# kepengxu/PGTFormer

Hardware: NVIDIA H100
Metric: clips_per_s (higher is better)
Workload: dtype bf16

## Files before the change

### pgtformer_b200/csrc/gemm_tc.cu

```cuda
#include <cudaTypedefs.h>
#include <cstdio>
#include <cstdlib>

#include "common.cuh"
#include "tmap.cuh"
#include "ptx.cuh"
#include "epi_common.cuh"

namespace pgt {

constexpr int BM = 128;
constexpr int BK = 64;
constexpr int EPI_WARPS = 8;
constexpr int GEMM_THREADS = EPI_WARPS * 32 + 128;
constexpr int PRODUCER_WARP = EPI_WARPS;
constexpr int DMA_WARP = EPI_WARPS + 1;
constexpr int CONSUMER_REGS = 232;
constexpr int PRODUCER_REGS = 40;
static_assert(2 * 128 * CONSUMER_REGS + 128 * PRODUCER_REGS <= 65536, "register file");
constexpr int XCH_LD = 68;
constexpr int XCH_BYTES = BM * XCH_LD * 4;
constexpr int XCH_WG_LD = 36;
constexpr int XCH_WG_BYTES = BM * XCH_WG_LD * 4;
constexpr int EPI_BAR = 1;
constexpr int PP_XCH_BAR = 2;
constexpr int PP_MMA_BAR = 4;
constexpr int PP_EPI_BAR = 6;
constexpr int A_STAGE_BYTES = BM * BK * 2;
constexpr int PANEL_BYTES = BM * 128;
template <int BN>
constexpr int staging_slots() { return BN == 256 ? 2 : 4; }
constexpr int PREFETCH_TILES = 2;

enum { MODE_LINEAR = 0, MODE_CONV_S1 = 1, MODE_CONV_S2 = 2 };

struct GemmParams {
  int mode;
  int M, N, K;
  int num_kb, m_tiles, n_tiles;
  int F, H, W;
  int tw, th, tn, tiles_x, tiles_y;
  int cin_blocks, ksize, pad_lo, cin_ld;
  int pad_x, pad_y;
  long long o_sx, o_sy, o_sf;
  int b_resident;
  int fast_epi;
  int has_res_map;
  const float* bias;
  int act, epi_mode;
  float* gn_stats;
  int gn_cpg;
  int ntaps, tap_kw, tap_oy, tap_ox;
  int gn_tpf;
  int gn_fstride;
  int relu_after_res;
  const void* residual;
  int ldr, res_dtype;
  const void* aux;
  int ldaux;
  float sft_w;
  void* out;
  int ldo, out_dtype, out_layout;
  double flops;
};

template <int BN>
struct GemmCfg {
  static constexpr int B_STAGE_BYTES = BN * BK * 2;
  static constexpr int STAGE_BYTES = A_STAGE_BYTES + B_STAGE_BYTES;
  static constexpr int SLOTS = staging_slots<BN>();
  static constexpr int STAGING_BYTES = SLOTS * PANEL_BYTES;
  static constexpr int BUDGET = 232448 - 1024  - STAGING_BYTES - XCH_BYTES - 256 ;
  static constexpr int STAGES = (BUDGET / STAGE_BYTES) > 6 ? 6 : (BUDGET / STAGE_BYTES);
  static constexpr int SMEM_BYTES = STAGES * STAGE_BYTES + STAGING_BYTES + XCH_BYTES + 256 + 1024;
  static_assert(SMEM_BYTES <= 232448, "gemm smem budget");
};

__device__ __forceinline__ void tile_mn(const GemmParams& p, int tile, int& m_blk, int& n_blk) {
  n_blk = tile % p.n_tiles;
  m_blk = tile / p.n_tiles;
}


__device__ __forceinline__ void decode_conv_tile(const GemmParams& p, int m_blk, int& n0, int& y0, int& x0) {
  const int tx = m_blk % p.tiles_x;
  const int t2 = m_blk / p.tiles_x;
  const int ty = t2 % p.tiles_y;
  const int tf = t2 / p.tiles_y;
  x0 = tx * p.tw;
  y0 = ty * p.th;
  n0 = tf * p.tn;
}

template <int N>
__device__ __forceinline__ void act_chunk(float (&f)[N], int act) {
  switch (act) {
    case PGT_ACT_GELU:
#pragma unroll
// ... 363 lines not shown
          mbar_wait_spin(&ctx.res_bar[pos], (k >> 1) & 1);
          const int col0 = col_base + pnl * PW + half * 32;
          uint32_t v[32];
          smem_row_32(xrow + half * 32, v);
          float4 nb[8];
          epi_finish<true>(p, v, bias_vec ? p.bias + col0 : nullptr, stg + pos * 2 * PANEL_BYTES, r, half, esize, true,
                           gn_ptr(col0), col0, nb, false);
          fence_proxy_async();
          mbar_arrive(&ctx.slot_ready[pos]);
          ++k;
        }
      } else {
        for (int pp = 0; pp < 64 / PW; ++pp) {
          const int pnl = g * (64 / PW) + pp;
          if (pnl >= npan) break;
          const int pos = k & (SLOTS - 1);
          const bool mine = (nsub == 2) || ((pnl & 1) == half);
          const int sb = (nsub == 2) ? half : 0;
          const int col0 = col_base + pnl * PW + sb * 32;
          float4 b[8];
          const bool pre = BN < 256 && bias_vec;
          if (mine && pre) {
            const float4* gb = reinterpret_cast<const float4*>(p.bias + col0);
#pragma unroll
            for (int q = 0; q < 8; ++q) b[q] = __ldg(gb + q);
          }
          mbar_wait_spin(&ctx.res_bar[pos], (k >> SLOT_SHIFT) & 1);
          if (mine) {
            uint32_t v[32];
            smem_row_32(xrow + pnl * PW + sb * 32 - g * 64, v);
            epi_finish<false>(p, v, bias_vec && !pre ? p.bias + col0 : nullptr, stg + pos * PANEL_BYTES, r, sb, esize,
                              p.has_res_map != 0, gn_ptr(col0), col0, b, pre);
          }
          fence_proxy_async();
          mbar_arrive(&ctx.slot_ready[pos]);
          ++k;
        }
      }
    } else {
      const int c0 = g * 64 + half * 32;
      if (drow.valid) {
#pragma unroll 1
        for (int sc16 = 0; sc16 < 32; sc16 += 16) {
          const int col0 = col_base + c0 + sc16;
          if (col0 >= p.N) break;
          epi_direct16(p, drow, xrow + half * 32 + sc16, col0);
        }
      }
      __syncwarp();
    }
  });
}

template <int BN>
__device__ __forceinline__ void epilogue_tile_wg(const GemmParams& p, const EpiCtx& ctx, int wq, int bar, int tile, int k,
                                                 const float (&acc)[2][BN / 2]) {
  const int lane = lane_id();
  const int r = wq * 32 + lane;
  const int esize = (p.out_dtype == PGT_BF16) ? 2 : 4;
  const ItemStream<BN> is(p, 0);
  const int nsub = is.PW / 32;
  constexpr int SLOTS = staging_slots<BN>();
  constexpr int SLOT_SHIFT = SLOTS == 4 ? 2 : 1;
  const bool sft = SLOTS == 4 && p.epi_mode == PGT_EPI_SFT;
  const bool bias_vec = p.bias != nullptr && (p.N % 32) == 0;
  const float* xrow = ctx.xch + r * XCH_WG_LD;

  int n_blk, m_blk;
  tile_mn(p, tile, m_blk, n_blk);
  const int col_base = n_blk * BN;
  const int npan = p.fast_epi ? is.panels_in_tile(tile) : 0;
  const uint32_t stg = smem_u32(ctx.staging) + r * 128;
  const DirectRow drow = p.fast_epi ? DirectRow{false, 0, 0, 0, 0} : direct_row(p, m_blk, r);

  static_for<0, BN / 32>([&](auto cc) {
    constexpr int c = decltype(cc)::value;
    const int pnl = c / nsub, sub = c - pnl * nsub;
    if (p.fast_epi && pnl >= npan) return;
    const int col0 = col_base + c * 32;
    if (col0 < p.N) {
      named_bar_sync(bar, 128);
      acc_to_smem<c * 32, 32>(acc[0], ctx.xch, XCH_WG_LD, wq, lane);
      acc_to_smem<c * 32, 32>(acc[1], ctx.xch + 64 * XCH_WG_LD, XCH_WG_LD, wq, lane);
      named_bar_sync(bar, 128);
    }
    if (p.fast_epi) {
      const int item = k + pnl;
      const int pos = sft ? (item & 1) : (item & (SLOTS - 1));
      if (sub == 0) mbar_wait_spin(&ctx.res_bar[pos], sft ? ((item >> 1) & 1) : ((item >> SLOT_SHIFT) & 1));
      if (col0 < p.N) {
        uint32_t v[32];
        smem_row_32(xrow, v);
        float4 nb[8];
        if (sft)
          epi_finish<true>(p, v, bias_vec ? p.bias + col0 : nullptr, stg + pos * 2 * PANEL_BYTES, r, sub, esize, true,
                           gn_stats_ptr(p, m_blk, wq, col0), col0, nb, false);
        else
          epi_finish<false>(p, v, bias_vec ? p.bias + col0 : nullptr, stg + pos * PANEL_BYTES, r, sub, esize,
                            p.has_res_map != 0, gn_stats_ptr(p, m_blk, wq, col0), col0, nb, false);
      }
      if (sub == nsub - 1) {
        fence_proxy_async();
        mbar_arrive(&ctx.slot_ready[pos]);
      }
    } else if (col0 < p.N) {
      if (drow.valid) {
#pragma unroll 1
        for (int sc16 = 0; sc16 < 32; sc16 += 16) {
          if (col0 + sc16 >= p.N) break;
          epi_direct16(p, drow, xrow + sc16, col0 + sc16);
        }
      }
      __syncwarp();
    }
  });
}

__device__ __forceinline__ void release_stage(uint64_t* bar, int lane) {
  __syncwarp();
  if (lane == 0) mbar_arrive(bar);
}

template <int BN>
__global__ void __launch_bounds__(GEMM_THREADS, 1)
gemm_tc_kernel(const __grid_constant__ CUtensorMap tmA, const __grid_constant__ CUtensorMap tmB,
               const __grid_constant__ CUtensorMap tmO, const __grid_constant__ CUtensorMap tmR,
               const __grid_constant__ CUtensorMap tmX, const GemmParams p) {
  using Cfg = GemmCfg<BN>;
  constexpr int STAGES = Cfg::STAGES;
  extern __shared__ uint8_t smem_raw[];
  uint8_t* smem = reinterpret_cast<uint8_t*>((reinterpret_cast<uintptr_t>(smem_raw) + 1023) & ~uintptr_t(1023));
  uint8_t* smem_a = smem;
  uint8_t* smem_b = smem + STAGES * A_STAGE_BYTES;
  uint8_t* staging = smem + STAGES * Cfg::STAGE_BYTES;
  float* xch = reinterpret_cast<float*>(staging + Cfg::STAGING_BYTES);
  uint64_t* bars = reinterpret_cast<uint64_t*>(staging + Cfg::STAGING_BYTES + XCH_BYTES);
  uint64_t* full_bar = bars;
  uint64_t* empty_bar = bars + STAGES;
  uint64_t* res_bar = bars + 2 * STAGES;
  uint64_t* slot_ready = res_bar + Cfg::SLOTS;

  const int warp = threadIdx.x >> 5;
  const int lane = threadIdx.x & 31;
  const int num_tiles = p.m_tiles * p.n_tiles;

  if (warp == PRODUCER_WARP && lane == 0) {
    tma_prefetch_desc(&tmA);
    tma_prefetch_desc(&tmB);
    if (p.fast_epi) tma_prefetch_desc(&tmO);
    if (p.has_res_map) tma_prefetch_desc(&tmR);
    if (p.fast_epi && p.epi_mode == PGT_EPI_SFT) tma_prefetch_desc(&tmX);
    for (int i = 0; i < STAGES; ++i) {
      mbar_init(&full_bar[i], 1);
      mbar_init(&empty_bar[i], EPI_WARPS);
    }
    for (int i = 0; i < Cfg::SLOTS; ++i) {
      mbar_init(&res_bar[i], 1);
      mbar_init(&slot_ready[i], EPI_WARPS * 32);
    }
    fence_barrier_init();
  }
  __syncthreads();

// ... 36 lines not shown
            tma_load_2d(dst_b, &tmB, &full_bar[stage], kb * BK, n_blk * BN);
          }
          __syncwarp();
          if (++stage == STAGES) { stage = 0; phase ^= 1; }
        }
      }
      for (int i = 0; i < STAGES; ++i) {
        mbar_wait(&empty_bar[stage], phase ^ 1);
        if (++stage == STAGES) { stage = 0; phase ^= 1; }
      }
    } else if (warp == DMA_WARP) {
      const EpiCtx ctx{staging, xch, res_bar, slot_ready};
      epilogue_dma_loop<BN>(p, ctx, tmO, tmR, tmX, lane, num_tiles);
    }
  } else {
    setmaxnreg_inc<CONSUMER_REGS>();
    const EpiCtx ctx{staging, xch, res_bar, slot_ready};
    const int wg = warp >> 2;
    const uint32_t a_rows = smem_u32(smem_a) + wg * 64 * 128;
    const uint32_t b_base = smem_u32(smem_b);
    int stage = 0;
    uint32_t phase = 0;
    int k = 0;
    for (int tile = blockIdx.x; tile < num_tiles; tile += gridDim.x) {
      float acc[BN / 2];
      int prev = -1;
      for (int kb = 0; kb < p.num_kb; ++kb) {
        mbar_wait_spin(&full_bar[stage], phase);
        const uint64_t da = wgmma_desc_k_sw128(a_rows + stage * A_STAGE_BYTES);
        const uint64_t db = wgmma_desc_k_sw128(b_base + stage * Cfg::B_STAGE_BYTES);
        wgmma_fence();
#pragma unroll
        for (int kk = 0; kk < BK / 16; ++kk)
          wgmma_bf16<BN>(acc, da + 2 * kk, db + 2 * kk, (kb | kk) != 0 ? 1u : 0u);
        wgmma_commit();
        wgmma_wait<1>();
        if (prev >= 0) release_stage(&empty_bar[prev], lane);
        prev = stage;
        if (++stage == STAGES) { stage = 0; phase ^= 1; }
      }
      wgmma_wait<0>();
      release_stage(&empty_bar[prev], lane);
      epilogue_tile<BN>(p, ctx, warp, lane, tile, k, acc);
    }
  }
}


constexpr int HALO_TW = 8, HALO_TH = 16;
constexpr int HALO_PITCH = (HALO_TW + 2) * 128;
constexpr int HALO_A_BYTES = (HALO_TH + 2) * HALO_PITCH;
constexpr int HALO_A_STRIDE = ((HALO_A_BYTES + 1023) / 1024) * 1024;

template <int BN>
struct HaloCfg {
  static constexpr int B_BYTES = BN * 128;
  static constexpr int A_STAGES = 2;
  static constexpr int B_STAGES = (BN == 64) ? 9 : 4;
  static constexpr int SLOTS = staging_slots<BN>();
  static constexpr int STAGING_BYTES = SLOTS * PANEL_BYTES;
  static constexpr int XCH = 2 * XCH_WG_BYTES;
  static constexpr int SMEM_BYTES = A_STAGES * HALO_A_STRIDE + B_STAGES * B_BYTES + STAGING_BYTES + XCH + 512 + 1024;
  static_assert(SMEM_BYTES <= 232448, "halo conv smem budget");
};

template <int S>
__device__ __forceinline__ void ring_skip(int& s, uint32_t& ph, int n) {
  const int t = s + n;
  ph ^= (uint32_t)(t / S) & 1u;
  s = t % S;
}

template <int BN>
__global__ void __launch_bounds__(GEMM_THREADS, 1)
conv_halo_kernel(const __grid_constant__ CUtensorMap tmA, const __grid_constant__ CUtensorMap tmB,
                 const __grid_constant__ CUtensorMap tmO, const __grid_constant__ CUtensorMap tmR,
                 const __grid_constant__ CUtensorMap tmX, const GemmParams p) {
  using Cfg = HaloCfg<BN>;
  constexpr int AS = Cfg::A_STAGES, BS = Cfg::B_STAGES;
  constexpr int RELEASERS = 4;
  extern __shared__ uint8_t smem_raw[];
  uint8_t* smem = reinterpret_cast<uint8_t*>((reinterpret_cast<uintptr_t>(smem_raw) + 1023) & ~uintptr_t(1023));
  uint8_t* smem_a = smem;
  uint8_t* smem_b = smem + AS * HALO_A_STRIDE;
  uint8_t* staging = smem_b + BS * Cfg::B_BYTES;
  float* xch = reinterpret_cast<float*>(staging + Cfg::STAGING_BYTES);
  uint64_t* bars = reinterpret_cast<uint64_t*>(staging + Cfg::STAGING_BYTES + Cfg::XCH);
  uint64_t* a_full = bars;
  uint64_t* a_empty = bars + AS;
  uint64_t* b_full = bars + 2 * AS;
  uint64_t* b_empty = bars + 2 * AS + BS;
  uint64_t* res_bar = bars + 2 * AS + 2 * BS;
  uint64_t* slot_ready = res_bar + Cfg::SLOTS;

  const int warp = threadIdx.x >> 5;
  const int lane = threadIdx.x & 31;
  const int num_tiles = p.m_tiles * p.n_tiles;
  const int cin_pad = p.cin_blocks * BK;

  if (warp == PRODUCER_WARP && lane == 0) {
    tma_prefetch_desc(&tmA);
    tma_prefetch_desc(&tmB);
    if (p.fast_epi) tma_prefetch_desc(&tmO);
    if (p.has_res_map) tma_prefetch_desc(&tmR);
    if (p.fast_epi && p.epi_mode == PGT_EPI_SFT) tma_prefetch_desc(&tmX);
    for (int i = 0; i < AS; ++i) { mbar_init(&a_full[i], 1); mbar_init(&a_empty[i], RELEASERS); }
    for (int i = 0; i < BS; ++i) { mbar_init(&b_full[i], 1); mbar_init(&b_empty[i], RELEASERS); }
    for (int i = 0; i < Cfg::SLOTS; ++i) {
      mbar_init(&res_bar[i], 1);
      mbar_init(&slot_ready[i], RELEASERS * 32);
    }
    fence_barrier_init();
  }
  __syncthreads();

  if (warp >= EPI_WARPS) {
    setmaxnreg_dec<PRODUCER_REGS>();
    if (warp == PRODUCER_WARP) {
      int as = 0, bs = 0;
      uint32_t aph = 0, bph = 0;
      for (int tile = blockIdx.x; tile < num_tiles; tile += gridDim.x) {
        const int n_blk = tile % p.n_tiles;
        const int m_blk = tile / p.n_tiles;
        int n0, y0, x0;
        decode_conv_tile(p, m_blk, n0, y0, x0);
        {
          const int pt = tile + PREFETCH_TILES * (int)gridDim.x;
          if (BN == 64 && pt < num_tiles && elect_one()) {
            int pn0, py0, px0;
            decode_conv_tile(p, pt / p.n_tiles, pn0, py0, px0);
            for (int cb = 0; cb < p.cin_blocks; ++cb) tma_prefetch_4d(&tmA, cb * BK, px0 - 1, py0 - 1, pn0);
            if (p.has_res_map) {
              const int c0 = (pt % p.n_tiles) * BN;
              const int rw = p.out_dtype == PGT_BF16 ? 64 : 32;
              for (int c = 0; c < BN && c0 + c < p.N; c += rw) {
                tma_prefetch_4d(&tmR, c0 + c, px0, py0, pn0);
                if (p.epi_mode == PGT_EPI_SFT) tma_prefetch_4d(&tmX, c0 + c, px0, py0, pn0);
              }
            }
          }
          __syncwarp();
        }
        for (int cb = 0; cb < p.cin_blocks; ++cb) {
          mbar_wait(&a_empty[as], aph ^ 1);
          if (elect_one()) {
            mbar_arrive_expect_tx(&a_full[as], HALO_A_BYTES);
            tma_load_4d(smem_a + as * HALO_A_STRIDE, &tmA, &a_full[as], cb * BK, x0 - 1, y0 - 1, n0);
          }
          __syncwarp();
          if (++as == AS) { as = 0; aph ^= 1; }
          if (p.b_resident && tile != (int)blockIdx.x) continue;
          for (int t = 0; t < p.ntaps; ++t) {
            mbar_wait(&b_empty[bs], bph ^ 1);
            if (elect_one()) {
              mbar_arrive_expect_tx(&b_full[bs], Cfg::B_BYTES);
              tma_load_2d(smem_b + bs * Cfg::B_BYTES, &tmB, &b_full[bs], t * cin_pad + cb * BK, n_blk * BN);
            }
            __syncwarp();
            if (++bs == BS) { bs = 0; bph ^= 1; }
          }
        }
      }
      for (int i = 0; i < AS; ++i) {
        mbar_wait(&a_empty[as], aph ^ 1);
        if (++as == AS) { as = 0; aph ^= 1; }
      }
    } else if (warp == DMA_WARP) {
      const EpiCtx ctx{staging, xch, res_bar, slot_ready};
      epilogue_dma_loop<BN>(p, ctx, tmO, tmR, tmX, lane, num_tiles);
    }
  } else {
    setmaxnreg_inc<CONSUMER_REGS>();
    const int wg = warp >> 2;
    const EpiCtx ctx{staging, xch + wg * (XCH_WG_BYTES / 4), res_bar, slot_ready};
    const uint32_t a_base = smem_u32(smem_a);
    const uint32_t b_base = smem_u32(smem_b);
    constexpr uint64_t ROW_BLOCK = 8 * HALO_PITCH / 16;
    const ItemStream<BN> is(p, num_tiles);
    const int b_per_tile = p.b_resident ? 0 : p.ntaps * p.cin_blocks;
    int as = 0, bs = 0;
    uint32_t aph = 0, bph = 0;
    int k = 0;
    bool first = true;
    for (int tile = blockIdx.x, j = 0; tile < num_tiles; tile += gridDim.x, ++j) {
      const bool has_next = tile + (int)gridDim.x < num_tiles;
      const int items = p.fast_epi ? is.panels_in_tile(tile) : 0;
      if ((j & 1) != wg) {
        ring_skip<AS>(as, aph, p.cin_blocks);
        ring_skip<BS>(bs, bph, b_per_tile);
        k += items;
        continue;
      }
      if (j > 0) named_bar_sync(PP_MMA_BAR + wg, 256);
      float acc[2][BN / 2];
      for (int cb = 0; cb < p.cin_blocks; ++cb) {
        const bool hand_over = has_next && cb == p.cin_blocks - 1;
        mbar_wait_spin(&a_full[as], aph);
        const uint64_t da0 = wgmma_desc_k_sw128(a_base + as * HALO_A_STRIDE, HALO_PITCH);
        auto tap_desc = [&](int t) -> uint64_t {
          const int dy = t / p.tap_kw, dx = t - dy * p.tap_kw;
          return da0 + (uint64_t)(((dy + p.tap_oy) * (HALO_TW + 2) + dx + p.tap_ox) * 8);
        };
        if (p.b_resident && first) {
          for (int t = 0; t < p.ntaps * p.cin_blocks; ++t) mbar_wait_spin(&b_full[t], 0);
          first = false;
        }
        int prev = -1;
        for (int t = 0; t < p.ntaps; ++t) {
          int bst = cb * p.ntaps + t;
          if (!p.b_resident) {
            mbar_wait_spin(&b_full[bs], bph);
            bst = bs;
          }
          const uint64_t da = tap_desc(t);
          const uint64_t db = wgmma_desc_k_sw128(b_base + bst * Cfg::B_BYTES);
          wgmma_fence();
#pragma unroll
          for (int kk = 0; kk < BK / 16; ++kk) {
            const uint32_t accum = (cb | t | kk) != 0 ? 1u : 0u;
            wgmma_bf16<BN>(acc[0], da + 2 * kk, db + 2 * kk, accum);
            wgmma_bf16<BN>(acc[1], da + ROW_BLOCK + 2 * kk, db + 2 * kk, accum);
          }
          wgmma_commit();
          if (hand_over && t == p.ntaps - 1) named_bar_arrive(PP_MMA_BAR + (wg ^ 1), 256);
          wgmma_wait<1>();
          if (!p.b_resident) {
            if (prev >= 0) release_stage(&b_empty[prev], lane);
            prev = bs;
            if (++bs == BS) { bs = 0; bph ^= 1; }
          }
        }
        wgmma_wait<0>();
        if (!p.b_resident) release_stage(&b_empty[prev], lane);
        release_stage(&a_empty[as], lane);
        if (++as == AS) { as = 0; aph ^= 1; }
      }
      if (j > 0) named_bar_sync(PP_EPI_BAR + wg, 256);
      epilogue_tile_wg<BN>(p, ctx, warp & 3, PP_XCH_BAR + wg, tile, k, acc);
      if (has_next) named_bar_arrive(PP_EPI_BAR + (wg ^ 1), 256);
      k += items;
    }
  }
}

static int encode_map(CUtensorMap* map, const void* base, int rank, const uint64_t* dims, const uint64_t* strides_bytes,
                      const uint32_t* box, int dtype = PGT_BF16) {
  return tmap_encode(map, base, rank, dims, strides_bytes, box, dtype);
}

static inline bool aligned16(const void* p) { return (reinterpret_cast<uintptr_t>(p) & 15) == 0; }

static int encode_out_map(CUtensorMap* map, const GemmParams& p, const void* base, int ld, int dtype) {
  const int esize = dtype == PGT_BF16 ? 2 : 4;
  const uint32_t pw = 128 / esize;
  if (p.mode == MODE_LINEAR) {
    uint64_t dims[2] = {(uint64_t)p.N, (uint64_t)p.M};
    uint64_t str[1] = {(uint64_t)ld * esize};
    uint32_t box[2] = {pw, BM};
    return encode_map(map, base, 2, dims, str, box, dtype);
  }
  uint64_t dims[4] = {(uint64_t)p.N, (uint64_t)p.W, (uint64_t)p.H, (uint64_t)p.F};
  uint64_t str[3] = {(uint64_t)ld * esize, (uint64_t)p.W * ld * esize, (uint64_t)p.H * p.W * ld * esize};
  if (p.o_sx != 0 && base == p.out) {
    str[0] = (uint64_t)p.o_sx * esize; str[1] = (uint64_t)p.o_sy * esize; str[2] = (uint64_t)p.o_sf * esize;
  }
  uint32_t box[4] = {pw, (uint32_t)p.tw, (uint32_t)p.th, (uint32_t)p.tn};
  return encode_map(map, base, 4, dims, str, box, dtype);
}

static int setup_epilogue_maps(GemmParams& p, const CUtensorMap& placeholder, CUtensorMap& tmO, CUtensorMap& tmR,
                               CUtensorMap& tmX) {
  const int esize = p.out_dtype == PGT_BF16 ? 2 : 4;
  p.fast_epi = (p.out_layout == PGT_OUT_NHWC && aligned16(p.out) && ((long long)p.ldo * esize) % 16 == 0) ? 1 : 0;
  if (p.epi_mode == PGT_EPI_SFT &&
      !(p.out_dtype == PGT_BF16 && aligned16(p.aux) && ((long long)p.ldaux * 2) % 16 == 0 && p.o_sx == 0))
    p.fast_epi = 0;
  p.has_res_map = 0;
  if (p.fast_epi && p.residual != nullptr) {
    if (p.res_dtype == p.out_dtype && aligned16(p.residual) && ((long long)p.ldr * esize) % 16 == 0) p.has_res_map = 1;
    else p.fast_epi = 0;
  }
  if (p.gn_stats != nullptr) {
    const int cpg = p.N / 32;
    const bool ok = p.fast_epi && p.out_dtype == PGT_BF16 && (p.N % 32) == 0 &&
                    (cpg == 2 || cpg == 4 || cpg == 8 || cpg == 16 || cpg == 32) &&
                    (p.mode == MODE_LINEAR || p.tn == 1);
    if (!ok) return PGT_ERR_UNSUPPORTED;
    p.gn_cpg = cpg;
  }
  tmO = placeholder;
  tmR = placeholder;
  tmX = placeholder;
  if (p.fast_epi) {
    int rc = encode_out_map(&tmO, p, p.out, p.ldo, p.out_dtype);
    if (rc != PGT_OK) return rc;
    if (p.has_res_map) {
      rc = encode_out_map(&tmR, p, p.residual, p.ldr, p.res_dtype);
      if (rc != PGT_OK) return rc;
    }
    if (p.epi_mode == PGT_EPI_SFT) {
      if (!p.has_res_map) { p.fast_epi = 0; return p.gn_stats ? PGT_ERR_UNSUPPORTED : PGT_OK; }
      rc = encode_out_map(&tmX, p, p.aux, p.ldaux, PGT_BF16);
      if (rc != PGT_OK) return rc;
    }
  }
  return PGT_OK;
}

static int encode_weight_map(CUtensorMap* tmB, const void* W, int ldw, int K, int N, int BN) {
  uint64_t dims[2] = {(uint64_t)K, (uint64_t)N};
  uint64_t str[1] = {(uint64_t)ldw * 2};
  uint32_t box[2] = {BK, (uint32_t)BN};
  return encode_map(tmB, W, 2, dims, str, box);
}

template <int BN>
static int launch_gemm(const CUtensorMap& tmA, const void* W, int ldw, GemmParams& p, cudaStream_t stream) {
  using Cfg = GemmCfg<BN>;
  static_assert(Cfg::STAGES >= 3, "pipeline too shallow");
  CUtensorMap tmB, tmO, tmR, tmX;
  int rc = encode_weight_map(&tmB, W, ldw, p.K, p.N, BN);
  if (rc != PGT_OK) return rc;
  rc = setup_epilogue_maps(p, tmA, tmO, tmR, tmX);
  if (rc != PGT_OK) return rc;
  p.n_tiles = ceil_div(p.N, BN);
  static PerDeviceOnce once;
  PGT_CUDA_OK(once.run([] { return cudaFuncSetAttribute(gemm_tc_kernel<BN>, cudaFuncAttributeMaxDynamicSharedMemorySize, Cfg::SMEM_BYTES); }));
  const int tiles = p.m_tiles * p.n_tiles;
  const int grid = tiles < num_sms() ? tiles : num_sms();
  {
    char desc[96];
    if (prof_enabled()) {
      if (p.mode == MODE_LINEAR) snprintf(desc, sizeof(desc), "linear M%d N%d K%d BN%d e%d", p.M, p.N, p.K, BN, p.fast_epi);
      else snprintf(desc, sizeof(desc), "conv%d s%d F%d H%d W%d K%d N%d BN%d t%dx%dx%d e%d", p.ksize, p.mode, p.F, p.H, p.W, p.K, p.N, BN, p.tn, p.th, p.tw, p.fast_epi);
    }
    ProfScope ps(PGT_PROF_GEMM, p.flops, stream, desc);
    gemm_tc_kernel<BN><<<grid, GEMM_THREADS, Cfg::SMEM_BYTES, stream>>>(tmA, tmB, tmO, tmR, tmX, p);
  }
  PGT_LAUNCH_OK();
  return PGT_OK;
}

template <int BN>
static int launch_halo(const CUtensorMap& tmA, const void* W, int ldw, GemmParams& p, cudaStream_t stream) {
  using Cfg = HaloCfg<BN>;
  CUtensorMap tmB, tmO, tmR, tmX;
  int rc = encode_weight_map(&tmB, W, ldw, p.K, p.N, BN);
  if (rc != PGT_OK) return rc;
  rc = setup_epilogue_maps(p, tmA, tmO, tmR, tmX);
  if (rc != PGT_OK) return rc;
  p.n_tiles = ceil_div(p.N, BN);
  p.b_resident = (p.ntaps * p.cin_blocks <= Cfg::B_STAGES && p.n_tiles == 1) ? 1 : 0;
  static PerDeviceOnce once;
  PGT_CUDA_OK(once.run([] { return cudaFuncSetAttribute(conv_halo_kernel<BN>, cudaFuncAttributeMaxDynamicSharedMemorySize, Cfg::SMEM_BYTES); }));
  const int tiles = p.m_tiles * p.n_tiles;
  const int grid = tiles < num_sms() ? tiles : num_sms();
  {
    char desc[96];
    if (prof_enabled())
      snprintf(desc, sizeof(desc), "halo3 F%d H%d W%d K%d N%d BN%d e%d r%d", p.F, p.H, p.W, p.K, p.N, BN, p.fast_epi,
               p.b_resident);
    ProfScope ps(PGT_PROF_GEMM, p.flops, stream, desc);
    conv_halo_kernel<BN><<<grid, GEMM_THREADS, Cfg::SMEM_BYTES, stream>>>(tmA, tmB, tmO, tmR, tmX, p);
  }
  PGT_LAUNCH_OK();
  return PGT_OK;
}

static bool wide_tiles(const GemmParams& p) {
  if (p.N <= 128 || p.num_kb < 8 || p.epi_mode == PGT_EPI_SFT) return false;
  if (ceil_div(p.N, 256) * 256 > ceil_div(p.N, 128) * 128) return false;
  return p.m_tiles * ceil_div(p.N, 256) >= num_sms();
}

static int dispatch_gemm(const CUtensorMap& tmA, const void* W, int ldw, GemmParams& p, cudaStream_t stream) {
  if (p.N <= 64) return launch_gemm<64>(tmA, W, ldw, p, stream);
  if (wide_tiles(p)) return launch_gemm<256>(tmA, W, ldw, p, stream);
  return launch_gemm<128>(tmA, W, ldw, p, stream);
}

static int fill_epilogue(GemmParams& p, const pgt_epilogue* ep) {
  if (ep == nullptr || ep->out == nullptr) return PGT_ERR_INVALID;
  p.bias = ep->bias;
  p.act = ep->act;
  p.epi_mode = ep->mode;
  p.residual = ep->residual;
  p.ldr = ep->ldr;
  p.res_dtype = ep->res_dtype;
  p.aux = ep->aux;
  p.ldaux = ep->ldaux;
  p.sft_w = ep->sft_w;
  p.out = ep->out;
  p.ldo = ep->ldo;
  p.out_dtype = ep->out_dtype;
  p.out_layout = ep->out_layout;
  p.relu_after_res = (ep->flags & PGT_EPI_FLAG_RELU_AFTER_RESIDUAL) ? 1 : 0;
  p.gn_stats = ep->gn_stats;
  p.gn_cpg = 0;
  if (p.relu_after_res && (p.act != PGT_ACT_RELU || p.epi_mode != PGT_EPI_PLAIN)) return PGT_ERR_INVALID;
  if (p.epi_mode == PGT_EPI_SFT && (p.residual == nullptr || p.aux == nullptr || p.res_dtype != PGT_BF16))
    return PGT_ERR_INVALID;
  if (p.out_layout == PGT_OUT_NCHW && (p.out_dtype != PGT_F32 || p.mode == MODE_LINEAR)) return PGT_ERR_INVALID;
  return PGT_OK;
}

}

using namespace pgt;

extern "C" int pgt_linear_bf16(const void* A, int lda, const void* W, int ldw, int M, int N, int K,
                               const pgt_epilogue* ep, void* stream) {
  PGT_CHECK_ARG(A && W && M > 0 && N > 0 && K > 0);
  PGT_CHECK_ARG((lda % 8) == 0 && (ldw % 8) == 0 && aligned16(A) && aligned16(W));
  GemmParams p{};
  p.mode = MODE_LINEAR;
  p.M = M; p.N = N; p.K = K;
  p.num_kb = ceil_div(K, BK);
  p.m_tiles = ceil_div(M, BM);
  p.flops = 2.0 * M * (double)N * K;
// ... 149 lines not shown
```

### pgtformer_b200/csrc/ptx.cuh

```cuda
#pragma once
#include <cuda_runtime.h>
#include <cuda.h>
#include <stdint.h>

#include <type_traits>

namespace pgt {

__device__ __forceinline__ uint32_t smem_u32(const void* p) {
  return static_cast<uint32_t>(__cvta_generic_to_shared(p));
}

__device__ __forceinline__ int lane_id() {
  int l;
  asm volatile("mov.u32 %0, %%laneid;" : "=r"(l));
  return l;
}

__device__ __forceinline__ bool elect_one() {
  uint32_t pred;
  asm volatile(
      "{\n\t.reg .pred P;\n\t"
      "elect.sync _|P, 0xffffffff;\n\t"
      "selp.u32 %0, 1, 0, P;\n\t}"
// ... 142 lines not shown
      : PGT_D8(0), PGT_D8(8)
      : "l"(da), "l"(db), "r"(acc));
}
__device__ __forceinline__ void wgmma_m64n48k16(float (&d)[24], uint64_t da, uint64_t db, uint32_t acc) {
  asm volatile(
      "{\n\t.reg .pred p;\n\tsetp.ne.b32 p, %26, 0;\n\t"
      "wgmma.mma_async.sync.aligned.m64n48k16.f32.bf16.bf16 {%0, %1, %2, %3, %4, %5, %6, %7, %8, %9, %10, %11, %12, %13, %14, %15, %16, %17, %18, %19, %20, %21, %22, %23}, %24, %25, p, 1, 1, 0, 0;\n\t}"
      : PGT_D24(0)
      : "l"(da), "l"(db), "r"(acc));
}
__device__ __forceinline__ void wgmma_m64n64k16(float (&d)[32], uint64_t da, uint64_t db, uint32_t acc) {
  asm volatile(
      "{\n\t.reg .pred p;\n\tsetp.ne.b32 p, %34, 0;\n\t"
      "wgmma.mma_async.sync.aligned.m64n64k16.f32.bf16.bf16 {%0, %1, %2, %3, %4, %5, %6, %7, %8, %9, %10, %11, %12, %13, %14, %15, %16, %17, %18, %19, %20, %21, %22, %23, %24, %25, %26, %27, %28, %29, %30, %31}, %32, %33, p, 1, 1, 0, 0;\n\t}"
      : PGT_D32(0)
      : "l"(da), "l"(db), "r"(acc));
}
__device__ __forceinline__ void wgmma_m64n128k16(float (&d)[64], uint64_t da, uint64_t db, uint32_t acc) {
  asm volatile(
      "{\n\t.reg .pred p;\n\tsetp.ne.b32 p, %66, 0;\n\t"
      "wgmma.mma_async.sync.aligned.m64n128k16.f32.bf16.bf16 {%0, %1, %2, %3, %4, %5, %6, %7, %8, %9, %10, %11, %12, %13, %14, %15, %16, %17, %18, %19, %20, %21, %22, %23, %24, %25, %26, %27, %28, %29, %30, %31, %32, %33, %34, %35, %36, %37, %38, %39, %40, %41, %42, %43, %44, %45, %46, %47, %48, %49, %50, %51, %52, %53, %54, %55, %56, %57, %58, %59, %60, %61, %62, %63}, %64, %65, p, 1, 1, 0, 0;\n\t}"
      : PGT_D64(0)
      : "l"(da), "l"(db), "r"(acc));
}
__device__ __forceinline__ void wgmma_m64n256k16(float (&d)[128], uint64_t da, uint64_t db, uint32_t acc) {
  asm volatile(
      "{\n\t.reg .pred p;\n\tsetp.ne.b32 p, %130, 0;\n\t"
      "wgmma.mma_async.sync.aligned.m64n256k16.f32.bf16.bf16 {%0, %1, %2, %3, %4, %5, %6, %7, %8, %9, %10, %11, %12, %13, %14, %15, %16, %17, %18, %19, %20, %21, %22, %23, %24, %25, %26, %27, %28, %29, %30, %31, %32, %33, %34, %35, %36, %37, %38, %39, %40, %41, %42, %43, %44, %45, %46, %47, %48, %49, %50, %51, %52, %53, %54, %55, %56, %57, %58, %59, %60, %61, %62, %63, %64, %65, %66, %67, %68, %69, %70, %71, %72, %73, %74, %75, %76, %77, %78, %79, %80, %81, %82, %83, %84, %85, %86, %87, %88, %89, %90, %91, %92, %93, %94, %95, %96, %97, %98, %99, %100, %101, %102, %103, %104, %105, %106, %107, %108, %109, %110, %111, %112, %113, %114, %115, %116, %117, %118, %119, %120, %121, %122, %123, %124, %125, %126, %127}, %128, %129, p, 1, 1, 0, 0;\n\t}"
      : PGT_D128(0)
      : "l"(da), "l"(db), "r"(acc));
}
template <int N>
__device__ __forceinline__ void wgmma_bf16(float (&d)[N / 2], uint64_t da, uint64_t db, uint32_t acc) {
  if constexpr (N == 16) wgmma_m64n16k16(d, da, db, acc);
  else if constexpr (N == 32) wgmma_m64n32k16(d, da, db, acc);
  else if constexpr (N == 48) wgmma_m64n48k16(d, da, db, acc);
  else if constexpr (N == 64) wgmma_m64n64k16(d, da, db, acc);
  else if constexpr (N == 128) wgmma_m64n128k16(d, da, db, acc);
  else { static_assert(N == 256, "wgmma N"); wgmma_m64n256k16(d, da, db, acc); }
}

__device__ __forceinline__ void wgmma_m64n64k16_rs_tb(float (&d)[32], const uint32_t (&a)[4], uint64_t db, uint32_t acc) {
  asm volatile(
      "{\n\t.reg .pred p;\n\tsetp.ne.b32 p, %37, 0;\n\t"
      "wgmma.mma_async.sync.aligned.m64n64k16.f32.bf16.bf16 {%0, %1, %2, %3, %4, %5, %6, %7, %8, %9, %10, %11, %12, %13, %14, %15, %16, %17, %18, %19, %20, %21, %22, %23, %24, %25, %26, %27, %28, %29, %30, %31}, {%32, %33, %34, %35}, %36, p, 1, 1, 1;\n\t}"
      : PGT_D32(0)
      : "r"(a[0]), "r"(a[1]), "r"(a[2]), "r"(a[3]), "l"(db), "r"(acc));
}
__device__ __forceinline__ void wgmma_m64n256k16_rs_tb(float (&d)[128], const uint32_t (&a)[4], uint64_t db, uint32_t acc) {
  asm volatile(
      "{\n\t.reg .pred p;\n\tsetp.ne.b32 p, %133, 0;\n\t"
      "wgmma.mma_async.sync.aligned.m64n256k16.f32.bf16.bf16 {%0, %1, %2, %3, %4, %5, %6, %7, %8, %9, %10, %11, %12, %13, %14, %15, %16, %17, %18, %19, %20, %21, %22, %23, %24, %25, %26, %27, %28, %29, %30, %31, %32, %33, %34, %35, %36, %37, %38, %39, %40, %41, %42, %43, %44, %45, %46, %47, %48, %49, %50, %51, %52, %53, %54, %55, %56, %57, %58, %59, %60, %61, %62, %63, %64, %65, %66, %67, %68, %69, %70, %71, %72, %73, %74, %75, %76, %77, %78, %79, %80, %81, %82, %83, %84, %85, %86, %87, %88, %89, %90, %91, %92, %93, %94, %95, %96, %97, %98, %99, %100, %101, %102, %103, %104, %105, %106, %107, %108, %109, %110, %111, %112, %113, %114, %115, %116, %117, %118, %119, %120, %121, %122, %123, %124, %125, %126, %127}, {%128, %129, %130, %131}, %132, p, 1, 1, 1;\n\t}"
      : PGT_D128(0)
      : "r"(a[0]), "r"(a[1]), "r"(a[2]), "r"(a[3]), "l"(db), "r"(acc));
}

template <int N>
__device__ __forceinline__ void setmaxnreg_dec() { asm volatile("setmaxnreg.dec.sync.aligned.u32 %0;" ::"n"(N)); }
template <int N>
__device__ __forceinline__ void setmaxnreg_inc() { asm volatile("setmaxnreg.inc.sync.aligned.u32 %0;" ::"n"(N)); }

__device__ __forceinline__ uint64_t wgmma_desc_mn_sw128(uint32_t saddr, uint32_t lbo = 16) {
  uint64_t d = 0;
  d |= static_cast<uint64_t>((saddr >> 4) & 0x3FFF);
  d |= static_cast<uint64_t>((lbo >> 4) & 0x3FFF) << 16;
  d |= static_cast<uint64_t>((1024 >> 4) & 0x3FFF) << 32;
  d |= static_cast<uint64_t>(1) << 62;
  return d;
}

template <int C0, int C, int R>
__device__ __forceinline__ void acc_to_smem(const float (&d)[R], float* scratch, int ld, int warp_in_wg, int lane) {
  static_assert(C0 % 8 == 0 && C % 8 == 0 && C0 + C <= 2 * R, "whole 8-column fragments inside D");
  const int row = 16 * warp_in_wg + (lane >> 2);
  float* p0 = scratch + row * ld + 2 * (lane & 3);
  float* p1 = p0 + 8 * ld;
#pragma unroll
  for (int j = 0; j < C / 8; ++j) {
    constexpr int f0 = C0 / 8;
    const int f = f0 + j;
    *reinterpret_cast<float2*>(p0 + 8 * j) = make_float2(d[4 * f + 0], d[4 * f + 1]);
    *reinterpret_cast<float2*>(p1 + 8 * j) = make_float2(d[4 * f + 2], d[4 * f + 3]);
  }
}

template <int I, int N, typename F>
__device__ __forceinline__ void static_for(F&& f) {
  if constexpr (I < N) {
    f(std::integral_constant<int, I>{});
    static_for<I + 1, N>(f);
  }
}

__device__ __forceinline__ void smem_row_32(const float* src, uint32_t (&v)[32]) {
#pragma unroll
  for (int q = 0; q < 8; ++q) {
    const float4 f = reinterpret_cast<const float4*>(src)[q];
    v[4 * q + 0] = __float_as_uint(f.x); v[4 * q + 1] = __float_as_uint(f.y);
    v[4 * q + 2] = __float_as_uint(f.z); v[4 * q + 3] = __float_as_uint(f.w);
  }
}

}
```

Before: 90.30.

## Add transposed halo conv kernel with register-resident weights for 64-channel convs

For 64-output-channel halo convolutions whose weights fit on chip, a new kernel variant keeps the weights in consumer registers as the wgmma A operand. It computes the transposed product (channels x 128 pixels) with m64n128 RS wgmma straight from the halo slab in shared memory. This removes the weight TMA ring, and the freed shared memory is spent on four A slab stages instead of two. The accumulator is written to shared memory transposed before the existing epilogue. The kernel also raises consumer register limits for the 9-tap case, which risks spills because weight fragments and 64 accumulators must fit in registers.

Result: faster. 92.40, median of 6 (+2.3%).

```diff
diff --git a/pgtformer_b200/csrc/gemm_tc.cu b/pgtformer_b200/csrc/gemm_tc.cu
--- a/pgtformer_b200/csrc/gemm_tc.cu
+++ b/pgtformer_b200/csrc/gemm_tc.cu
@@ -18,6 +18,9 @@
 constexpr int CONSUMER_REGS = 232;
 constexpr int PRODUCER_REGS = 40;
 static_assert(2 * 128 * CONSUMER_REGS + 128 * PRODUCER_REGS <= 65536, "register file");
+constexpr int T9_CONSUMER_REGS = 240;
+constexpr int T9_PRODUCER_REGS = 24;
+static_assert(2 * 128 * T9_CONSUMER_REGS + 128 * T9_PRODUCER_REGS <= 168 * 384, "register pool of the launch bound");
 constexpr int XCH_LD = 68;
 constexpr int XCH_BYTES = BM * XCH_LD * 4;
 constexpr int XCH_WG_LD = 36;
@@ -44,6 +47,8 @@
   int pad_x, pad_y;
   long long o_sx, o_sy, o_sf;
   int b_resident;
+  const __nv_bfloat16* w;
+  int ldw;
   int fast_epi;
   int has_res_map;
   const float* bias;
@@ -513,9 +518,10 @@
   });
 }
 
-template <int BN>
+template <int BN, bool kT, typename Acc>
 __device__ __forceinline__ void epilogue_tile_wg(const GemmParams& p, const EpiCtx& ctx, int wq, int bar, int tile, int k,
-                                                 const float (&acc)[2][BN / 2]) {
+                                                 const Acc& acc) {
+  static_assert(!kT || BN == 64, "the transposed accumulator holds 64 channels");
   const int lane = lane_id();
   const int r = wq * 32 + lane;
   const int esize = (p.out_dtype == PGT_BF16) ? 2 : 4;
@@ -525,7 +531,12 @@
   constexpr int SLOT_SHIFT = SLOTS == 4 ? 2 : 1;
   const bool sft = SLOTS == 4 && p.epi_mode == PGT_EPI_SFT;
   const bool bias_vec = p.bias != nullptr && (p.N % 32) == 0;
-  const float* xrow = ctx.xch + r * XCH_WG_LD;
+  const float* xrow = ctx.xch + r * (kT ? XCH_LD : XCH_WG_LD);
+  if constexpr (kT) {
+    named_bar_sync(bar, 128);
+    acc_t_to_smem(acc, ctx.xch, XCH_LD, wq, lane);
+    named_bar_sync(bar, 128);
+  }
 
   int n_blk, m_blk;
   tile_mn(p, tile, m_blk, n_blk);
@@ -539,11 +550,14 @@
     const int pnl = c / nsub, sub = c - pnl * nsub;
     if (p.fast_epi && pnl >= npan) return;
     const int col0 = col_base + c * 32;
-    if (col0 < p.N) {
-      named_bar_sync(bar, 128);
-      acc_to_smem<c * 32, 32>(acc[0], ctx.xch, XCH_WG_LD, wq, lane);
-      acc_to_smem<c * 32, 32>(acc[1], ctx.xch + 64 * XCH_WG_LD, XCH_WG_LD, wq, lane);
-      named_bar_sync(bar, 128);
+    const float* xc = kT ? xrow + c * 32 : xrow;
+    if constexpr (!kT) {
+      if (col0 < p.N) {
+        named_bar_sync(bar, 128);
+        acc_to_smem<c * 32, 32>(acc[0], ctx.xch, XCH_WG_LD, wq, lane);
+        acc_to_smem<c * 32, 32>(acc[1], ctx.xch + 64 * XCH_WG_LD, XCH_WG_LD, wq, lane);
+        named_bar_sync(bar, 128);
+      }
     }
     if (p.fast_epi) {
       const int item = k + pnl;
@@ -551,7 +565,7 @@
       if (sub == 0) mbar_wait_spin(&ctx.res_bar[pos], sft ? ((item >> 1) & 1) : ((item >> SLOT_SHIFT) & 1));
       if (col0 < p.N) {
         uint32_t v[32];
-        smem_row_32(xrow, v);
+        smem_row_32(xc, v);
         float4 nb[8];
         if (sft)
           epi_finish<true>(p, v, bias_vec ? p.bias + col0 : nullptr, stg + pos * 2 * PANEL_BYTES, r, sub, esize, true,
@@ -569,7 +583,7 @@
 #pragma unroll 1
         for (int sc16 = 0; sc16 < 32; sc16 += 16) {
           if (col0 + sc16 >= p.N) break;
-          epi_direct16(p, drow, xrow + sc16, col0 + sc16);
+          epi_direct16(p, drow, xc + sc16, col0 + sc16);
         }
       }
       __syncwarp();
@@ -712,14 +726,14 @@
 constexpr int HALO_A_BYTES = (HALO_TH + 2) * HALO_PITCH;
 constexpr int HALO_A_STRIDE = ((HALO_A_BYTES + 1023) / 1024) * 1024;
 
-template <int BN>
+template <int BN, bool kT = false>
 struct HaloCfg {
   static constexpr int B_BYTES = BN * 128;
-  static constexpr int A_STAGES = 2;
-  static constexpr int B_STAGES = (BN == 64) ? 9 : 4;
+  static constexpr int A_STAGES = kT ? 4 : 2;
+  static constexpr int B_STAGES = kT ? 0 : (BN == 64) ? 9 : 4;
   static constexpr int SLOTS = staging_slots<BN>();
   static constexpr int STAGING_BYTES = SLOTS * PANEL_BYTES;
-  static constexpr int XCH = 2 * XCH_WG_BYTES;
+  static constexpr int XCH = kT ? 2 * XCH_BYTES : 2 * XCH_WG_BYTES;
   static constexpr int SMEM_BYTES = A_STAGES * HALO_A_STRIDE + B_STAGES * B_BYTES + STAGING_BYTES + XCH + 512 + 1024;
   static_assert(SMEM_BYTES <= 232448, "halo conv smem budget");
 };
@@ -731,12 +745,14 @@
   s = t % S;
 }
 
-template <int BN>
+template <int BN, int TAPS = 0, int CBLK = 0>
 __global__ void __launch_bounds__(GEMM_THREADS, 1)
 conv_halo_kernel(const __grid_constant__ CUtensorMap tmA, const __grid_constant__ CUtensorMap tmB,
                  const __grid_constant__ CUtensorMap tmO, const __grid_constant__ CUtensorMap tmR,
                  const __grid_constant__ CUtensorMap tmX, const GemmParams p) {
-  using Cfg = HaloCfg<BN>;
+  constexpr bool kT = TAPS > 0;
+  static_assert(!kT || (BN == 64 && TAPS * CBLK <= 9), "transposed: 64 channels, at most 9 resident weight blocks");
+  using Cfg = HaloCfg<BN, kT>;
   constexpr int AS = Cfg::A_STAGES, BS = Cfg::B_STAGES;
   constexpr int RELEASERS = 4;
   extern __shared__ uint8_t smem_raw[];
@@ -775,7 +791,7 @@
   __syncthreads();
 
   if (warp >= EPI_WARPS) {
-    setmaxnreg_dec<PRODUCER_REGS>();
+    setmaxnreg_dec<TAPS == 9 ? T9_PRODUCER_REGS : PRODUCER_REGS>();
     if (warp == PRODUCER_WARP) {
       int as = 0, bs = 0;
       uint32_t aph = 0, bph = 0;
@@ -809,15 +825,17 @@
           }
           __syncwarp();
           if (++as == AS) { as = 0; aph ^= 1; }
-          if (p.b_resident && tile != (int)blockIdx.x) continue;
-          for (int t = 0; t < p.ntaps; ++t) {
-            mbar_wait(&b_empty[bs], bph ^ 1);
-            if (elect_one()) {
-              mbar_arrive_expect_tx(&b_full[bs], Cfg::B_BYTES);
-              tma_load_2d(smem_b + bs * Cfg::B_BYTES, &tmB, &b_full[bs], t * cin_pad + cb * BK, n_blk * BN);
+          if constexpr (!kT) {
+            if (p.b_resident && tile != (int)blockIdx.x) continue;
+            for (int t = 0; t < p.ntaps; ++t) {
+              mbar_wait(&b_empty[bs], bph ^ 1);
+              if (elect_one()) {
+                mbar_arrive_expect_tx(&b_full[bs], Cfg::B_BYTES);
+                tma_load_2d(smem_b + bs * Cfg::B_BYTES, &tmB, &b_full[bs], t * cin_pad + cb * BK, n_blk * BN);
+              }
+              __syncwarp();
+              if (++bs == BS) { bs = 0; bph ^= 1; }
             }
-            __syncwarp();
-            if (++bs == BS) { bs = 0; bph ^= 1; }
           }
         }
       }
@@ -829,7 +847,7 @@
       const EpiCtx ctx{staging, xch, res_bar, slot_ready};
       epilogue_dma_loop<BN>(p, ctx, tmO, tmR, tmX, lane, num_tiles);
     }
-  } else {
+  } else if constexpr (!kT) {
     setmaxnreg_inc<CONSUMER_REGS>();
     const int wg = warp >> 2;
     const EpiCtx ctx{staging, xch + wg * (XCH_WG_BYTES / 4), res_bar, slot_ready};
@@ -896,9 +914,73 @@
         if (++as == AS) { as = 0; aph ^= 1; }
       }
       if (j > 0) named_bar_sync(PP_EPI_BAR + wg, 256);
-      epilogue_tile_wg<BN>(p, ctx, warp & 3, PP_XCH_BAR + wg, tile, k, acc);
+      epilogue_tile_wg<BN, false>(p, ctx, warp & 3, PP_XCH_BAR + wg, tile, k, acc);
       if (has_next) named_bar_arrive(PP_EPI_BAR + (wg ^ 1), 256);
       k += items;
+    }
+  } else {
+    setmaxnreg_inc<TAPS == 9 ? T9_CONSUMER_REGS : CONSUMER_REGS>();
+    constexpr int KW = TAPS == 9 ? 3 : 2;
+    uint32_t wf[CBLK * TAPS * 4][4];
+    {
+      const int m0 = 16 * (warp & 3) + (lane >> 2), m1 = m0 + 8, c0 = 2 * (lane & 3);
+      const __nv_bfloat16* w0 = p.w + (size_t)m0 * p.ldw + c0;
+      const __nv_bfloat16* w1 = p.w + (size_t)m1 * p.ldw + c0;
+      auto ld = [](const __nv_bfloat16* q) { return __ldg(reinterpret_cast<const unsigned int*>(q)); };
+#pragma unroll
+      for (int cb = 0; cb < CBLK; ++cb)
+#pragma unroll
+        for (int t = 0; t < TAPS; ++t)
+#pragma unroll
+          for (int kk = 0; kk < BK / 16; ++kk) {
+            const int col = t * cin_pad + cb * BK + kk * 16;
+            uint32_t(&a)[4] = wf[(cb * TAPS + t) * 4 + kk];
+            a[0] = m0 < p.N ? ld(w0 + col) : 0u;
+            a[1] = m1 < p.N ? ld(w1 + col) : 0u;
+            a[2] = m0 < p.N ? ld(w0 + col + 8) : 0u;
+            a[3] = m1 < p.N ? ld(w1 + col + 8) : 0u;
+          }
+    }
+    auto base = [&]() {
+      uint8_t* b;
+      asm volatile("mov.b64 %0, %1;" : "=l"(b) : "l"(smem));
+      return b;
+    };
+    constexpr int BARS = AS * HALO_A_STRIDE + Cfg::STAGING_BYTES + Cfg::XCH;
+    static_assert((AS & (AS - 1)) == 0, "slab ring position from the tile count");
+    for (int tile = blockIdx.x, j = 0; tile < num_tiles; tile += gridDim.x, ++j) {
+      if ((j & 1) != (warp >> 2)) continue;
+      if (j > 0) named_bar_sync(PP_MMA_BAR + (warp >> 2), 256);
+      float acc[64];
+#pragma unroll
+      for (int cb = 0; cb < CBLK; ++cb) {
+        const int as = (j * CBLK + cb) & (AS - 1);
+        const uint32_t aph = ((j * CBLK + cb) / AS) & 1;
+        uint64_t* a_bars = reinterpret_cast<uint64_t*>(base() + BARS);
+        mbar_wait_spin(&a_bars[as], aph);
+        const uint64_t db0 = wgmma_desc_k_sw128(smem_u32(base()) + as * HALO_A_STRIDE, HALO_PITCH) +
+                             (uint64_t)((p.tap_oy * (HALO_TW + 2) + p.tap_ox) * 8);
+        wgmma_fence();
+#pragma unroll
+        for (int t = 0; t < TAPS; ++t) {
+          const uint64_t db = db0 + (uint64_t)(((t / KW) * (HALO_TW + 2) + t % KW) * 8);
+#pragma unroll
+          for (int kk = 0; kk < BK / 16; ++kk)
+            wgmma_m64n128k16_rs(acc, wf[(cb * TAPS + t) * 4 + kk], db + 2 * kk, (cb | t | kk) != 0 ? 1u : 0u);
+        }
+        wgmma_commit();
+        if (cb == CBLK - 1 && tile + (int)gridDim.x < num_tiles) named_bar_arrive(PP_MMA_BAR + ((warp >> 2) ^ 1), 256);
+        wgmma_wait<0>();
+        release_stage(&a_bars[AS + as], lane_id());
+      }
+      const int wg = warp >> 2;
+      uint8_t* b = base();
+      uint64_t* res = reinterpret_cast<uint64_t*>(b + BARS) + 2 * AS;
+      const EpiCtx ctx{b + AS * HALO_A_STRIDE, reinterpret_cast<float*>(b + AS * HALO_A_STRIDE + Cfg::STAGING_BYTES) +
+                                                   wg * (XCH_BYTES / 4),
+                       res, res + Cfg::SLOTS};
+      const int k = p.fast_epi ? j * ItemStream<BN>(p, num_tiles).panels_in_tile(tile) : 0;
+      epilogue_tile_wg<BN, true>(p, ctx, warp & 3, PP_XCH_BAR + wg, tile, k, acc);
     }
   }
 }
@@ -1001,30 +1083,46 @@
   return PGT_OK;
 }
 
+template <int BN, int TAPS = 0, int CBLK = 0>
+static int launch_halo_kernel(const CUtensorMap& tmA, const CUtensorMap& tmB, const CUtensorMap& tmO,
+                              const CUtensorMap& tmR, const CUtensorMap& tmX, const GemmParams& p, cudaStream_t stream) {
+  using Cfg = HaloCfg<BN, (TAPS > 0)>;
+  static PerDeviceOnce once;
+  PGT_CUDA_OK(once.run([] {
+    return cudaFuncSetAttribute(conv_halo_kernel<BN, TAPS, CBLK>, cudaFuncAttributeMaxDynamicSharedMemorySize, Cfg::SMEM_BYTES);
+  }));
+  const int tiles = p.m_tiles * p.n_tiles;
+  const int grid = tiles < num_sms() ? tiles : num_sms();
+  {
+    char desc[96];
+    if (prof_enabled())
+      snprintf(desc, sizeof(desc), "halo3 F%d H%d W%d K%d N%d BN%d e%d r%d T%d", p.F, p.H, p.W, p.K, p.N, BN, p.fast_epi,
+               p.b_resident, TAPS > 0 ? 1 : 0);
+    ProfScope ps(PGT_PROF_GEMM, p.flops, stream, desc);
+    conv_halo_kernel<BN, TAPS, CBLK><<<grid, GEMM_THREADS, Cfg::SMEM_BYTES, stream>>>(tmA, tmB, tmO, tmR, tmX, p);
+  }
+  PGT_LAUNCH_OK();
+  return PGT_OK;
+}
+
 template <int BN>
 static int launch_halo(const CUtensorMap& tmA, const void* W, int ldw, GemmParams& p, cudaStream_t stream) {
-  using Cfg = HaloCfg<BN>;
   CUtensorMap tmB, tmO, tmR, tmX;
   int rc = encode_weight_map(&tmB, W, ldw, p.K, p.N, BN);
   if (rc != PGT_OK) return rc;
   rc = setup_epilogue_maps(p, tmA, tmO, tmR, tmX);
   if (rc != PGT_OK) return rc;
   p.n_tiles = ceil_div(p.N, BN);
-  p.b_resident = (p.ntaps * p.cin_blocks <= Cfg::B_STAGES && p.n_tiles == 1) ? 1 : 0;
-  static PerDeviceOnce once;
-  PGT_CUDA_OK(once.run([] { return cudaFuncSetAttribute(conv_halo_kernel<BN>, cudaFuncAttributeMaxDynamicSharedMemorySize, Cfg::SMEM_BYTES); }));
-  const int tiles = p.m_tiles * p.n_tiles;
-  const int grid = tiles < num_sms() ? tiles : num_sms();
-  {
-    char desc[96];
-    if (prof_enabled())
-      snprintf(desc, sizeof(desc), "halo3 F%d H%d W%d K%d N%d BN%d e%d r%d", p.F, p.H, p.W, p.K, p.N, BN, p.fast_epi,
-               p.b_resident);
-    ProfScope ps(PGT_PROF_GEMM, p.flops, stream, desc);
-    conv_halo_kernel<BN><<<grid, GEMM_THREADS, Cfg::SMEM_BYTES, stream>>>(tmA, tmB, tmO, tmR, tmX, p);
-  }
-  PGT_LAUNCH_OK();
-  return PGT_OK;
+  p.b_resident = (p.ntaps * p.cin_blocks <= HaloCfg<BN>::B_STAGES && p.n_tiles == 1) ? 1 : 0;
+  if (BN == 64 && p.b_resident) {
+    p.w = static_cast<const __nv_bfloat16*>(W);
+    p.ldw = ldw;
+    if (p.ntaps == 9) return launch_halo_kernel<64, 9, 1>(tmA, tmB, tmO, tmR, tmX, p, stream);
+    if (p.ntaps == 4 && p.cin_blocks == 1) return launch_halo_kernel<64, 4, 1>(tmA, tmB, tmO, tmR, tmX, p, stream);
+    if (p.ntaps == 4 && p.cin_blocks == 2) return launch_halo_kernel<64, 4, 2>(tmA, tmB, tmO, tmR, tmX, p, stream);
+    return PGT_ERR_UNSUPPORTED;
+  }
+  return launch_halo_kernel<BN>(tmA, tmB, tmO, tmR, tmX, p, stream);
 }
 
 static bool wide_tiles(const GemmParams& p) {
diff --git a/pgtformer_b200/csrc/ptx.cuh b/pgtformer_b200/csrc/ptx.cuh
--- a/pgtformer_b200/csrc/ptx.cuh
+++ b/pgtformer_b200/csrc/ptx.cuh
@@ -218,6 +218,14 @@
       "{\n\t.reg .pred p;\n\tsetp.ne.b32 p, %133, 0;\n\t"
       "wgmma.mma_async.sync.aligned.m64n256k16.f32.bf16.bf16 {%0, %1, %2, %3, %4, %5, %6, %7, %8, %9, %10, %11, %12, %13, %14, %15, %16, %17, %18, %19, %20, %21, %22, %23, %24, %25, %26, %27, %28, %29, %30, %31, %32, %33, %34, %35, %36, %37, %38, %39, %40, %41, %42, %43, %44, %45, %46, %47, %48, %49, %50, %51, %52, %53, %54, %55, %56, %57, %58, %59, %60, %61, %62, %63, %64, %65, %66, %67, %68, %69, %70, %71, %72, %73, %74, %75, %76, %77, %78, %79, %80, %81, %82, %83, %84, %85, %86, %87, %88, %89, %90, %91, %92, %93, %94, %95, %96, %97, %98, %99, %100, %101, %102, %103, %104, %105, %106, %107, %108, %109, %110, %111, %112, %113, %114, %115, %116, %117, %118, %119, %120, %121, %122, %123, %124, %125, %126, %127}, {%128, %129, %130, %131}, %132, p, 1, 1, 1;\n\t}"
       : PGT_D128(0)
+      : "r"(a[0]), "r"(a[1]), "r"(a[2]), "r"(a[3]), "l"(db), "r"(acc));
+}
+
+__device__ __forceinline__ void wgmma_m64n128k16_rs(float (&d)[64], const uint32_t (&a)[4], uint64_t db, uint32_t acc) {
+  asm volatile(
+      "{\n\t.reg .pred p;\n\tsetp.ne.b32 p, %69, 0;\n\t"
+      "wgmma.mma_async.sync.aligned.m64n128k16.f32.bf16.bf16 {%0, %1, %2, %3, %4, %5, %6, %7, %8, %9, %10, %11, %12, %13, %14, %15, %16, %17, %18, %19, %20, %21, %22, %23, %24, %25, %26, %27, %28, %29, %30, %31, %32, %33, %34, %35, %36, %37, %38, %39, %40, %41, %42, %43, %44, %45, %46, %47, %48, %49, %50, %51, %52, %53, %54, %55, %56, %57, %58, %59, %60, %61, %62, %63}, {%64, %65, %66, %67}, %68, p, 1, 1, 0;\n\t}"
+      : PGT_D64(0)
       : "r"(a[0]), "r"(a[1]), "r"(a[2]), "r"(a[3]), "l"(db), "r"(acc));
 }
 
@@ -250,6 +258,18 @@
   }
 }
 
+__device__ __forceinline__ void acc_t_to_smem(const float (&d)[64], float* scratch, int ld, int warp_in_wg, int lane) {
+  float* p0 = scratch + 2 * (lane & 3) * ld + 16 * warp_in_wg + (lane >> 2);
+#pragma unroll
+  for (int j = 0; j < 16; ++j) {
+    float* q = p0 + 8 * j * ld;
+    q[0] = d[4 * j + 0];
+    q[ld] = d[4 * j + 1];
+    q[8] = d[4 * j + 2];
+    q[ld + 8] = d[4 * j + 3];
+  }
+}
+
 template <int I, int N, typename F>
 __device__ __forceinline__ void static_for(F&& f) {
   if constexpr (I < N) {
```
